# NethermindEth/latticefold

Hardware: AMD Instinct MI355X
Metric: folding-prover steps/sec (one NIFSProver::prove per step), GoldilocksRingNTT (higher is better)
Workload: dtype u64; 1 GPU; C4: GoldilocksRingNTT R1CS->CCS, m=N=2^20 rows, wit_len=262144, L=4, B=2^16, b=2, K=16, kappa=26, t=3; parallelism=replicas x1

## Files before the change

latticefold_amd/csrc/lf_common.h:

```cpp
#pragma once
#include <hip/hip_runtime.h>

#include <stdlib.h>

#include <atomic>

#include "../../include/lfhip.h"

#define HIPCHK(x)                                    \
    do {                                             \
        hipError_t e__ = (x);                        \
        if (e__ != hipSuccess) return LF_ERR_HIP;    \
    } while (0)
#define RET(x)                      \
    do {                            \
        int rc__ = (x);             \
        if (rc__ != LF_OK) return rc__; \
    } while (0)

extern "C" void lfplus_scratch_trim(int device);
template <class T> static inline hipError_t lf_dev_malloc(T **p, size_t bytes) {
    hipError_t e = hipMalloc((void **)p, bytes);
    if (e != hipErrorOutOfMemory) return e;
    (void)hipGetLastError();
    int dev = 0;
    if (hipGetDevice(&dev) != hipSuccess) return e;
    lfplus_scratch_trim(dev);
    return hipMalloc((void **)p, bytes);
}

struct DevBuf {
    void *p = nullptr;
    size_t bytes = 0;
    int ensure(size_t b) {
        if (b <= bytes) return LF_OK;
        if (p) (void)hipFree(p);
        p = nullptr;
        bytes = 0;
        const size_t slack = (b >> 3) < ((size_t)8 << 20) ? (b >> 3) : ((size_t)8 << 20);
        size_t want = b + slack + 256;
        if (hipMalloc(&p, want) != hipSuccess) {
            if (lf_dev_malloc(&p, b) != hipSuccess) return LF_ERR_HIP;
            want = b;
        }
        bytes = want;
        return LF_OK;
    }
    void release() {
        if (p) (void)hipFree(p);
        p = nullptr;
        bytes = 0;
    }
};

inline uint64_t lf_next_witness_id() {
    static std::atomic<uint64_t> next{1};
    return next.fetch_add(1, std::memory_order_relaxed);
}
struct lf_witness {
    lf_ctx *ctx;
    int32_t *planes;
    size_t N;
    int device;
    size_t plane_bytes;
    uint64_t id = lf_next_witness_id();
    uint64_t *f_ntt = nullptr;
    size_t f_bytes = 0;
    uint64_t *w_ccs = nullptr;
    size_t w_bytes = 0;
};

int lf_planes_alloc(lf_ctx *ctx, size_t bytes, int32_t **out);
void lf_planes_release(lf_ctx *ctx, size_t bytes, int32_t *p);
int lf_ctx_device(const lf_ctx *ctx);


struct Tunables {
    bool lin_u_eval = false, fold_unfused = false, fold_no_lut = false, fold_tab_r1 = false, theta_eval = false, fold_no_r4tab = false, fold_no_r5tab = false;
    bool fold_rounds_no_split = false;
    bool fold_sv_no_split = false;
    bool lin_no_split = false;
    size_t lin_split_min = (size_t)1 << 17;
    size_t fold_split_min = 8192;
    bool force_exchange = false;
    bool device_transcript = false;
    bool shard_plain_rounds = false;
    int shard_two_lanes = -1;
    size_t shard_lin_min = 16384;
    size_t shard_fold_min = 2048;
    long i8_wgs = 0;
    bool lin_no_r1cs = false;
    bool lin_no_small = false;
    size_t dot_min = 4096;
    bool dot_valu = false;
    bool fold_no_sv = false;
    size_t sv_min = 65536;
    int sv_rounds = 3;
    bool no_tail = false;
    size_t fuse_min = 16384, lut_min = (size_t)1 << 17, tab_min = 16384;
    size_t r5_min = 8192;
    size_t tail_n = 2048;
    static Tunables read(size_t lut_min_default) {
        Tunables t;
        t.lut_min = lut_min_default;
        const char *e;
        t.lin_u_eval = getenv("LF_LIN_U_EVAL") != nullptr;
        t.fold_unfused = getenv("LF_FOLD_UNFUSED") != nullptr;
        t.fold_no_lut = getenv("LF_FOLD_NO_LUT") != nullptr;
        t.fold_tab_r1 = getenv("LF_FOLD_TAB_R1") != nullptr;
        t.fold_no_r4tab = getenv("LF_FOLD_NO_R4TAB") != nullptr;
        t.fold_no_r5tab = getenv("LF_FOLD_NO_R5TAB") != nullptr;
        t.lin_no_split = getenv("LF_LIN_NO_SPLIT") != nullptr;
        t.fold_sv_no_split = getenv("LF_FOLD_SV_NO_SPLIT") != nullptr;
        t.fold_rounds_no_split = getenv("LF_FOLD_ROUNDS_NO_SPLIT") != nullptr;
        if (const char *e = getenv("LF_LIN_SPLIT_MIN")) t.lin_split_min = (size_t)atoll(e);
        if (const char *e = getenv("LF_FOLD_SPLIT_MIN")) t.fold_split_min = (size_t)atoll(e);
        t.theta_eval = getenv("LF_THETA_EVAL") != nullptr;
        t.no_tail = getenv("LF_NO_TAIL") != nullptr;
        t.fold_no_sv = getenv("LF_FOLD_NO_SV") != nullptr;
        t.dot_valu = getenv("LF_DOT_VALU") != nullptr;
        if ((e = getenv("LF_DOT_MIN"))) t.dot_min = (size_t)atoll(e);
        t.lin_no_small = getenv("LF_LIN_NO_SMALL") != nullptr;
        t.lin_no_r1cs = getenv("LF_LIN_NO_R1CS") != nullptr;
        if ((e = getenv("LF_FOLD_SV_MIN"))) t.sv_min = (size_t)atoll(e);
        if ((e = getenv("LF_FOLD_SV_ROUNDS"))) t.sv_rounds = atoi(e);
        if ((e = getenv("LF_I8_WGS"))) t.i8_wgs = atol(e);
        if ((e = getenv("LF_SHARD_TWO_LANES"))) t.shard_two_lanes = atoi(e) != 0;
        if ((e = getenv("LF_SHARD_LIN_MIN"))) t.shard_lin_min = (size_t)atoll(e);
        if ((e = getenv("LF_SHARD_FOLD_MIN"))) t.shard_fold_min = (size_t)atoll(e);
        t.shard_plain_rounds = getenv("LF_SHARD_PLAIN_ROUNDS") != nullptr;
        t.device_transcript = getenv("LF_DEVICE_TRANSCRIPT") != nullptr;
        t.force_exchange = getenv("LF_DIST_FORCE_EXCHANGE") != nullptr;
        if ((e = getenv("LF_FOLD_FUSE_MIN"))) t.fuse_min = (size_t)atoll(e);
        if ((e = getenv("LF_FOLD_LUT_MIN"))) t.lut_min = (size_t)atoll(e);
        if ((e = getenv("LF_FOLD_TAB_MIN"))) t.tab_min = (size_t)atoll(e);
        if ((e = getenv("LF_TAIL_N"))) t.tail_n = (size_t)atoll(e);
        if ((e = getenv("LF_FOLD_R5_MIN"))) t.r5_min = (size_t)atoll(e);
        return t;
    }
};

static inline int lf_validate_csr(unsigned t, size_t m, size_t n, const uint32_t *const *rowptr, const uint32_t *const *col,
                                  const uint64_t *const *val, int words, uint64_t modulus) {
    for (unsigned j = 0; j < t; j++) {
        if (!rowptr[j] || !col[j] || !val[j]) return LF_ERR_INVALID;
        if (rowptr[j][0] != 0) return LF_ERR_INVALID;
        for (size_t r = 0; r < m; r++)
            if (rowptr[j][r + 1] < rowptr[j][r]) return LF_ERR_INVALID;
        const size_t nnz = rowptr[j][m];
        for (size_t k = 0; k < nnz; k++)
            if (col[j][k] >= n) return LF_ERR_INVALID;
        for (size_t k = 0; k < nnz * (size_t)words; k++)
            if (val[j][k] >= modulus) return LF_ERR_INVALID;
    }
    return LF_OK;
}

struct ExtBasis {
    bool on = false;
    int tau = 0;
    uint64_t p = 0;
    uint64_t T[81], Ti[81];
    static uint64_t mulmod(uint64_t a, uint64_t b, uint64_t p) { return (uint64_t)(((unsigned __int128)a * b) % p); }
    void apply(const uint64_t *M, uint64_t *v) const {
        uint64_t o[9];
        for (int i = 0; i < tau; i++) {
            unsigned __int128 acc = 0;
            for (int j = 0; j < tau; j++) acc += (unsigned __int128)mulmod(M[i * tau + j], v[j], p);
            o[i] = (uint64_t)(acc % p);
        }
        for (int i = 0; i < tau; i++) v[i] = o[i];
    }
    void to_ext(uint64_t *v, size_t slots) const { if (on) for (size_t s = 0; s < slots; s++) apply(T, v + s * tau); }
    void to_int(uint64_t *v, size_t slots) const { if (on) for (size_t s = 0; s < slots; s++) apply(Ti, v + s * tau); }
    int set(const uint64_t *Tin, int tau_, uint64_t p_) {
        tau = tau_; p = p_;
        uint64_t M[9][18];
        bool ident = true;
        for (int i = 0; i < tau; i++)
            for (int j = 0; j < tau; j++) {
                uint64_t v = Tin[i * tau + j] % p;
                T[i * tau + j] = v; M[i][j] = v; M[i][tau + j] = i == j;
                if (v != (uint64_t)(i == j)) ident = false;
            }
        for (int i = 0; i < tau; i++)
            if (T[i * tau] != (uint64_t)(i == 0)) return LF_ERR_BAD_TABLES;
        auto inv = [&](uint64_t a) { uint64_t r = 1, e = p - 2; while (e) { if (e & 1) r = mulmod(r, a, p); a = mulmod(a, a, p); e >>= 1; } return r; };
        for (int c = 0; c < tau; c++) {
            int piv = -1;
            for (int r = c; r < tau; r++) if (M[r][c]) { piv = r; break; }
            if (piv < 0) return LF_ERR_BAD_TABLES;
            if (piv != c) for (int k = 0; k < 2 * tau; k++) { uint64_t t = M[piv][k]; M[piv][k] = M[c][k]; M[c][k] = t; }
            uint64_t iv = inv(M[c][c]);
            for (int k = 0; k < 2 * tau; k++) M[c][k] = mulmod(M[c][k], iv, p);
            for (int r = 0; r < tau; r++) {
                if (r == c || !M[r][c]) continue;
                uint64_t f = M[r][c];
                for (int k = 0; k < 2 * tau; k++) { uint64_t t = mulmod(f, M[c][k], p); M[r][k] = M[r][k] >= t ? M[r][k] - t : M[r][k] + (p - t); }
            }
        }
        for (int i = 0; i < tau; i++)
            for (int j = 0; j < tau; j++) Ti[i * tau + j] = M[i][tau + j];
// ... 5 lines not shown
```

latticefold_amd/csrc/lf_fold.cpp:

```cpp
#include "lf_ctx.h"

static int upload_consts(lf_ctx *c, const std::string &name, const std::vector<Fq3Const> &v, Fq3Const **out) {
    RET(c->tbuf(name, v.size() + 8, out));
    return c->h2d_small(*out, v.data(), v.size() * sizeof(Fq3Const));
}

static int tail_host_rounds(lf_ctx *c, Transcript &tr, u32 epoch, u32 nr, u32 npts, bool dev_transcript, u64 *msgs, Fq3 *pt,
                            const std::function<void(u32)> *after_round = nullptr, u32 round0 = 0) {
    TailMail *mail = c->tail_mail;
    const auto t_start = std::chrono::steady_clock::now();
    double host_us = 0, wait_us = 0;
    auto t_mark = t_start;
    const bool tl_on = t_tl && t_tl->on;
    for (u32 i = 0; i < nr; i++) {
        u32 spins = 0;
        while (__atomic_load_n(&mail->msg_seq[i], __ATOMIC_ACQUIRE) != epoch) {
            __builtin_ia32_pause();
            if ((++spins & 0xfff) == 0) {
                if (__atomic_load_n(&mail->err, __ATOMIC_RELAXED) == epoch ||
                    std::chrono::duration<double>(std::chrono::steady_clock::now() - t_start).count() > 10.0) {
                    __atomic_store_n(&mail->abort_seq, epoch, __ATOMIC_RELEASE);
                    (void)hipStreamSynchronize(c->stream());
                    return LF_ERR_HIP;
                }
// ... 83 lines not shown
    auto find = [&](unsigned s, unsigned b) {
        for (int i = 0; i < NPR; i++)
            if (prs[i].s == s && prs[i].b == b) return i;
        return -1;
    };
    std::vector<Fq3> wa(NX), wb(NX);
    for (int x = 0; x < NX; x++) {
        if (x < V) { wa[x] = W[x]; wb[x] = fq3_neg(W[x]); }
        else { wa[x] = fq3_zero(); wb[x] = W[x - V]; }
    }
    for (int x = 0; x < NX; x++)
        for (int y = x; y < NX; y++) {
            const Fq3 p2[3] = {c->ring.mul3(wa[x], wa[y]), fq3_add(c->ring.mul3(wa[x], wb[y]), c->ring.mul3(wb[x], wa[y])), c->ring.mul3(wb[x], wb[y])};
            for (int z = y; z < NX; z++) {
                Fq3 p3[4];
                p3[0] = c->ring.mul3(p2[0], wa[z]);
                p3[1] = fq3_add(c->ring.mul3(p2[0], wb[z]), c->ring.mul3(p2[1], wa[z]));
                p3[2] = fq3_add(c->ring.mul3(p2[1], wb[z]), c->ring.mul3(p2[2], wa[z]));
                p3[3] = c->ring.mul3(p2[2], wb[z]);
                int mult, idx;
                if (x == y && y == z) { mult = 1; idx = find(1u << x, 1u << x); }
                else if (x == y) { mult = 3; idx = find(1u << z, (1u << x) | (1u << z)); }
                else if (y == z) { mult = 3; idx = find(1u << x, (1u << x) | (1u << y)); }
                else { mult = 6; const unsigned mk = (1u << x) | (1u << y) | (1u << z); idx = find(mk, mk); }
                for (int e = 0; e < 4; e++) {
                    Fq3 t = p3[e], acc = fq3_zero();
                    for (int i = 0; i < mult; i++) acc = fq3_add(acc, t);
                    C[(size_t)idx * 4 + e] = fq3_add(C[(size_t)idx * 4 + e], acc);
                }
            }
        }
    for (int x = 0; x < NX; x++) {
        const int idx = find(1u << x, 1u << x);
        C[(size_t)idx * 4] = fq3_sub(C[(size_t)idx * 4], wa[x]);
        C[(size_t)idx * 4 + 1] = fq3_sub(C[(size_t)idx * 4 + 1], wb[x]);
    }
    out.resize((size_t)NPR * 12);
    for (size_t i = 0; i < (size_t)NPR * 4; i++)
        for (int q = 0; q < 3; q++) out[i * 3 + q] = C[i].c[q];
}

int fold_impl(lf_ctx *c, Transcript &tr, SideState *S , u64 *lcccs_out, lf_witness **w_out, u64 *proof) {
    const lf_params &P = c->P;
    size_t m = c->m, n = c->n, N = c->N;
    u32 K = P.K, K2 = 2 * K, deg = 2 * P.b;
    size_t ll = lf_lcccs_len(&P);
    std::vector<Fq3> alpha(K2), zeta(K2), mu(K2), beta(P.s);
    {
        HostTimer ht(c);
        tr.absorb_label("alpha_s");
        for (u32 i = 0; i < K2; i++) alpha[i] = tr.get_challenge();
        tr.absorb_label("zeta_s");
        for (u32 i = 0; i < K2; i++) zeta[i] = tr.get_challenge();
    }
    size_t ph = c->ev_begin(13);
    std::vector<Fq3Const> mu_pow((size_t)K2 * 3), a_pow((size_t)K2 * 3), z_pow((size_t)K2 * P.t);
    for (u32 i = 0; i < K2; i++) {
        Fq3 pa = alpha[i], pz = zeta[i];
        for (u32 d = 0; d < 3; d++) { a_pow[(size_t)i * 3 + d] = f3c(pa); pa = c->ring.mul3(pa, alpha[i]); }
        for (u32 j = 0; j < P.t; j++) { z_pow[(size_t)i * P.t + j] = f3c(pz); pz = c->ring.mul3(pz, zeta[i]); }
    }
    Fq3Const *d_mu, *d_ap, *d_zp;
    RET(upload_consts(c, "c_ap", a_pow, &d_ap));
    RET(upload_consts(c, "c_zp", z_pow, &d_zp));
    u64 *G[2], *eqb, *zz, *partial, *od;
    RET(c->tbuf("fold_G1", 24 * m, &G[0]));
    RET(c->tbuf("fold_G2", 24 * m, &G[1]));
    RET(c->tbuf("fold_eqb", 3 * m, &eqb));
    RET(c->tbuf("fold_zz", (size_t)P.t * 24 * n, &zz));
    RET(c->tbuf("round_partial", round_partial_words(), &partial));
    od = c->round_out();
    if (!od) return LF_ERR_HIP;
    u64 *const od_host = od, *od_shard = nullptr;
    if (c->sh_world > 1) {
        RET(c->tbuf("fold_round_out", 5 * 24 + 8, &od_shard));
        od = od_shard;
    }
    const bool shard_tabs = shard_keep(c, 1, m);
    const size_t g_r0 = shard_tabs ? (size_t)c->sh_rank * (m / (size_t)c->sh_world) : 0, g_rcnt = shard_tabs ? m / (size_t)c->sh_world : (size_t)-1;
    size_t zc_lo = 0, zc_hi = n;
    if (shard_tabs) RET(shard_col_range(c, g_r0, g_rcnt, &zc_lo, &zc_hi));
    {
        hipStream_t s0 = c->stream(), s1 = (t_lane == 0) ? c->st_lane[1] : s0;
        u64 *zz1 = zz;
        if (s1 != s0) {
            RET(c->tbuf("fold_zz1", (size_t)P.t * 24 * n, &zz1));
            if (!c->ev_prep[0]) { HIPCHK(hipEventCreateWithFlags(&c->ev_prep[0], hipEventDisableTiming)); HIPCHK(hipEventCreateWithFlags(&c->ev_prep[1], hipEventDisableTiming)); }
            HIPCHK(hipEventRecord(c->ev_prep[0], s0));
            HIPCHK(hipStreamWaitEvent(s1, c->ev_prep[0], 0));
        }
        for (int sd = 0; sd < 2; sd++) {
            hipStream_t st = sd ? s1 : s0;
            u64 *zb = sd ? zz1 : zz;
            launch_lincomb_z(c->dcrt, S[sd].z + zc_lo, n, K, d_zp + (size_t)sd * K * P.t, P.t, zc_hi - zc_lo, zb + zc_lo, st);
            if (c->ccs_general) {
                u64 *zaos;
                RET(c->tbuf(sd ? "spmv_zaos_R" : "spmv_zaos_L", (size_t)P.t * n * 24, &zaos));
                launch_spmv_rows(c->dcrt, P.t, c->d_rowptr.data(), c->d_col.data(), c->d_val.data(), zb, (size_t)24 * n, n, zaos, G[sd], m, 0, st, g_r0, g_rcnt);
            } else
            launch_spmv_sum(c->dcrt, P.t, c->d_rowptr.data(), c->d_col.data(), c->d_val.data(), zb, (size_t)24 * n, n, G[sd], m, st, g_r0, g_rcnt);
            launch_add_fhat_comb(c->dcrt, S[sd].planes, N, K, d_ap + (size_t)sd * K * 3, G[sd], m, st, g_r0, g_rcnt);
        }
        if (s1 != s0) {
            HIPCHK(hipEventRecord(c->ev_prep[1], s1));
            HIPCHK(hipStreamWaitEvent(s0, c->ev_prep[1], 0));
        }
    }
    {
        HostTimer ht(c);
        tr.absorb_label("mu_s");
        for (u32 i = 0; i + 1 < K2; i++) mu[i] = tr.get_challenge();
        mu[K2 - 1] = fq3_one();
        tr.absorb_label("beta_s");
        for (u32 i = 0; i < P.s; i++) beta[i] = tr.get_challenge();
    }
    TL_MARK(" fold challenges");
    for (u32 i = 0; i < K2; i++) {
        Fq3 pm = mu[i];
        for (u32 d = 0; d < 3; d++) { mu_pow[(size_t)i * 3 + d] = f3c(pm); pm = c->ring.mul3(pm, mu[i]); }
    }
    RET(upload_consts(c, "c_mu", mu_pow, &d_mu));
    RET(build_eq_dev(c, beta.data(), P.s, eqb));
    u64 *svE[3] = {nullptr, nullptr, nullptr};
    const bool sv_split = !c->tn.fold_sv_no_split && P.s >= 4 && m >= 256;
    if (sv_split) {
        RET(c->tbuf("fold_svE1", 3 * (m / 2), &svE[0]));
        RET(c->tbuf("fold_svE2", 3 * (m / 4), &svE[1]));
        RET(c->tbuf("fold_svE3", 3 * (m / 8), &svE[2]));
        RET(build_eq_dev(c, beta.data() + 1, P.s - 1, svE[0]));
    }
    Fq3 sv_c = fq3_one();
    u32 svE_level = 1;
    const bool fr_split = sv_split && c->sh_world == 1 && c->dcrt.nu2p40 && !c->tn.fold_rounds_no_split;
    u64 *svE_rest = nullptr;
    if (fr_split) RET(c->tbuf("fold_svE_rest", 3 * (m / 8) + 64, &svE_rest));
    auto svE_ptr = [&](u32 l) -> u64 * {
        if (l <= 3) return svE[l - 1];
        size_t off = 0;
        for (u32 q = 4; q < l; q++) off += 3 * (m >> q);
        return svE_rest + off;
    };
    auto svE_ensure = [&](u32 l) {
        for (; svE_level < l; svE_level++)
            launch_eq_pairsum(svE_ptr(svE_level), m >> svE_level, m >> (svE_level + 1), svE_ptr(svE_level + 1), m >> (svE_level + 1), c->stream());
    };
    auto sv_c_at = [&](u32 round, const std::vector<Fq3> &ptv) {
        Fq3 cc = fq3_one();
        for (u32 k = 1; k < round; k++) {
            const Fq3 b = beta[k - 1], r = ptv[k - 1];
            cc = c->ring.mul3(cc, fq3_add(c->ring.mul3(fq3_sub(fq3_one(), b), fq3_sub(fq3_one(), r)), c->ring.mul3(b, r)));
        }
        return cc;
    };
    LF_TRACE(c, "fold prepare");
    c->ev_end(ph);
    if (t_tl && t_tl->on) { (void)hipStreamSynchronize(c->stream()); TL_MARK(" fold prepare (synced)"); }

    ph = c->ev_begin(14);
    u64 *msgs = proof;
    std::vector<Fq3> pt(P.s);
    { HostTimer ht(c); sc_prologue(tr, P.s, deg); }
    const size_t Gw = (size_t)c->sh_world, gr = (size_t)c->sh_rank;
    bool sharded = Gw > 1;
    const bool fused = !c->tn.fold_unfused && (Gw == 1 || !c->tn.shard_plain_rounds);
    const size_t fuse_min = c->tn.fuse_min;
    int fmode = 0;
    const u64 *prevF = nullptr;
    size_t prevld = 0;
    const size_t lut_min = c->tn.lut_min;
    const size_t tab_min = c->tn.tab_min;
    const bool use_lut = fused && P.s >= 4 && m / 4 >= lut_min && m / 4 >= 4 && !c->tn.fold_no_lut;
    const bool use_r4tab = use_lut && c->dcrt.nu2p40 && !c->tn.fold_no_r4tab;
    const bool use_r5 = use_r4tab && !c->tn.fold_no_r5tab && Gw == 1 && P.s >= 5 && (N & 3) == 0 && (c->tn.no_tail || m / 8 > c->tn.tail_n) && m / 32 >= c->tn.r5_min;
    u64 *F[2], *T5[2];
    size_t half = m / 2;
    const size_t f0_ent = use_lut ? m / 16 : m / 4, f1_ent = use_r5 ? m / 32 : m / 8;
    RET(c->tbuf("fold_F0", (size_t)K2 * 3 * 24 * (f0_ent ? f0_ent : 1), &F[0]));
// ... 662 lines not shown
```

latticefold_amd/csrc/lf_kernels.h:

```cpp
#pragma once
#include "lf_ajtai_i8.h"
#include "lf_sv_rounds.h"
#include <hip/hip_runtime.h>

#include "lf_host.h"

namespace lf {

struct DevCrt {
    u64 nu;
    int nu2p40;
    u64 w4, w2, w10, w1, w7, w5, w11;
    int slot_of_pos[8], pos1[8], pos2[8];
    u64 tw1[8], tw2[8];
};
DevCrt make_dev_crt(const CrtTables &T);

struct Fq3Const { u64 c[3]; };

void launch_aos_to_soa(const u64 *aos, u64 *soa, size_t n, hipStream_t s);
void launch_soa_to_aos(const u64 *soa, u64 *aos, size_t n, hipStream_t s);
void launch_fill_uniform(u64 *dst, size_t words, u64 seed, size_t start, hipStream_t s);
void launch_fill_ajtai(u64 *A, u32 kappa, size_t n, size_t n_total, size_t col0, u64 seed, hipStream_t s, u32 row0 = 0);

void launch_modsum(const u64 *parts, u32 nparts, size_t words, u64 *out, hipStream_t s);
void launch_gather_relayout(const u64 *all, u32 nranks, size_t planes, size_t lcl, u64 *full, hipStream_t s);
void launch_gather_relayout_part(const u64 *all, u32 nranks, size_t planes_tot, size_t p0, size_t planes, size_t lcl, u64 *full, hipStream_t s);

void launch_selftest_field(u64 seed, u32 n, u64 *mism_dev, hipStream_t s);

void launch_crt_fwd(const DevCrt &t, const u64 *coef, u64 *ntt, size_t n, hipStream_t s);
void launch_icrt_dense(const u64 *icrt_mat , const u64 *ntt, u64 *coef, size_t n, hipStream_t s);


void launch_decompose(const u64 *coef, size_t n, u64 base, u32 digits, int layout, u64 *out, hipStream_t s, int mode = 0);
void launch_recompose(const u64 *in, size_t n_out, u64 base, u32 digits, u64 *out, hipStream_t s);
void launch_coef_to_i32(const u64 *coef, int32_t *planes, size_t n, u32 bound, int *viol, hipStream_t s);
void launch_i32_to_coef(const int32_t *planes, u64 *coef, size_t n, hipStream_t s);
void launch_recompose_crt(const DevCrt &t, const int32_t *planes, size_t n_planes, u32 wit_len, u32 L, u64 B, u32 K,
                          int mode_bits, u64 *out, size_t ldz, size_t off, hipStream_t s);
void launch_linf(const u64 *coef, size_t n, u64 *out_max, hipStream_t s);


void launch_build_eq(const DevCrt &t, const Fq3Const *r_dev , u32 nv, u64 *eq , hipStream_t s);
size_t build_eq_scratch_words(u32 nv);
void launch_build_eq2(const DevCrt &t, const Fq3Const *r_dev, u32 nv, u64 *scratch, u64 *eq, hipStream_t s);
void launch_spmv(const DevCrt &t, const u32 *rowptr, const u32 *col, const u64 *val , const u64 *z,
                 size_t ldz, u64 *out, size_t m, int accumulate, hipStream_t s, size_t r0 = 0, size_t rcnt = (size_t)-1 );
void launch_spmv_sum(const DevCrt &t, u32 nm, const u32 *const *rowptr, const u32 *const *col, const u64 *const *val, const u64 *z,
                     size_t z_stride, size_t ldz, u64 *out, size_t m, hipStream_t s, size_t r0 = 0, size_t rcnt = (size_t)-1 );
void launch_spmv_rows(const DevCrt &t, u32 nm, const u32 *const *rowptr, const u32 *const *col, const u64 *const *val, const u64 *z, size_t z_stride, size_t n,
                      u64 *zaos, u64 *out, size_t m, int accumulate, hipStream_t s, size_t r0 = 0, size_t rcnt = (size_t)-1);
void launch_spmv_t_eq(const DevCrt &t, const u32 *colptr, const u32 *rowidx, const u64 *val, const u64 *eq, size_t m,
                      u64 *q, size_t n, hipStream_t s, size_t c0 = 0, size_t ccnt = (size_t)-1 );
void launch_dot_batch(const DevCrt &t, const u64 *X, size_t ldx, u32 na, const u64 *Y, size_t ldy, u32 nb, size_t n,
                      u64 *partial, u64 *out, hipStream_t s);
size_t dot_partial_words(u32 na, u32 nb);
void launch_dot_eq(const DevCrt &t, const u64 *X, size_t ldx, u32 na, const u64 *eq, size_t ldeq, size_t n, u64 *partial,
                   u64 *out, hipStream_t s);
void launch_coef_eval(const DevCrt &t, const int32_t *planes, size_t n, const u64 *eq, size_t ldeq, u32 K, int mode_bits,
                      u64 *partial, u64 *out, hipStream_t s, size_t ldp = 0);
size_t coef_eval_partial_words(u32 K);
void launch_lincomb_z(const DevCrt &t, const u64 *z, size_t ldz, u32 K, const Fq3Const *coef_dev , u32 tt, size_t n,
                      u64 *out, hipStream_t s, u32 per_slot = 0);
void launch_add_fhat_comb(const DevCrt &t, const int32_t *planes, size_t n_planes, u32 K, const Fq3Const *apow_dev ,
                          u64 *G, size_t m, hipStream_t s, size_t r0 = 0, size_t rcnt = (size_t)-1 );

void launch_fix_ring(const DevCrt &t, const u64 *in, u64 *out, size_t n_in, Fq3Const r, hipStream_t s);
void launch_fix_fq3(const DevCrt &t, const u64 *in, u64 *out, size_t n_in, Fq3Const r, hipStream_t s);
size_t dot_i8_yb_bytes(size_t n);
size_t dot_i8_part_words(size_t n);
size_t dot_i8_tot_words();
int launch_dot_batch_i8(const DevCrt &t, const u64 *X, size_t ldx, u32 na, const u64 *Y, size_t ldy, u32 nb, size_t n, unsigned char *YB, int32_t *part,
                        long long *tot, u64 *out, hipStream_t s, bool y_packed = false, u32 nb_out = 0, u32 b0 = 0);
int launch_dot_pack_y(const u64 *X, const u64 *Y, size_t ldy, u32 nb, size_t n, unsigned char *YB, hipStream_t s);
void launch_vs_combine(const u64 *vs , u32 K, u64 *v , hipStream_t s);
void launch_fix_final(const DevCrt &t, const u64 *in , u32 rows3, Fq3Const r, u64 *out , hipStream_t s);

struct LinCombDesc {
    u32 t, q;
    u32 S_off[9];
    u32 S_idx[16];
    u64 c[8][24];
    int c_unit[8];
    u32 first[4];
    u32 ms[4];
};
void launch_lin_round(const DevCrt &t, const LinCombDesc &desc, const u64 *mz, size_t ld, const u64 *eq, size_t ldeq, size_t n,
                      u32 deg, u64 *partial, u64 *out, hipStream_t s, u32 max_blocks = 0, u32 split_xmask = 0 );
void launch_lin_round_fused(const DevCrt &t, const LinCombDesc &desc, const u64 *mz_prev, size_t ld_prev, const u64 *eq_prev, size_t ldeq_prev, Fq3Const r, u64 *mz_out,
                            size_t ld_out, u64 *eq_out, size_t ldeq_out, size_t n, u32 deg, u64 *partial, u64 *out, hipStream_t s, u32 max_blocks = 0,
                            u32 split_xmask = 0 );
void launch_eq_pairsum(const u64 *in, size_t ld_in, size_t n_out, u64 *out, size_t ld_out, hipStream_t s);
void launch_eq_expand(const DevCrt &t, const u64 *E, size_t lde, size_t pairs, Fq3Const w0, Fq3Const w1, u64 *out, size_t ldo, hipStream_t s);

struct FoldRoundArgs {
    const u64 *eqL, *eqR, *eqB;
    const u64 *G1, *G2;
    size_t ld;
    size_t n;
    size_t p0, pcnt;
    size_t pF0;
};
void launch_fold_round1(const DevCrt &t, const FoldRoundArgs &a, const int32_t *planesL, const int32_t *planesR, size_t n_planes,
                        u32 K, const Fq3Const *mu_pow_dev , u64 *partial, u64 *out, hipStream_t s);
void launch_fold_round_g(const DevCrt &t, const FoldRoundArgs &a, u64 *partial, u64 *out, hipStream_t s);
void launch_fold_materialize(const DevCrt &t, const int32_t *planesL, const int32_t *planesR, size_t n_planes, size_t m, u32 K,
                             Fq3Const r1, u64 *F, hipStream_t s);
void launch_fold_round2(const DevCrt &t, const FoldRoundArgs &a, const int32_t *planesL, const int32_t *planesR, size_t n_planes, u32 K,
                        const Fq3Const *mu_pow_dev, Fq3Const r1, u64 *partial, u64 *out, hipStream_t s);
void launch_fold_round_tab(const DevCrt &t, int round, const FoldRoundArgs &a, const int32_t *planesL, const int32_t *planesR, size_t n_planes, u32 K,
                           const Fq3Const *mu_pow_dev, const u64 *poly_dev, u64 *tp_dev, u64 *partial, u64 *out, hipStream_t s);
void launch_fold_materialize2(const DevCrt &t, const int32_t *planesL, const int32_t *planesR, size_t n_planes, size_t j0, size_t q, u32 K,
                              const Fq3Const W[4], u64 *F, hipStream_t s);
void launch_fold_round(const DevCrt &t, const FoldRoundArgs &a, const u64 *F, size_t ldF, u32 K, const Fq3Const *mu_pow_dev,
                       u64 *partial, u64 *out, hipStream_t s);
void launch_fold_round_lut_fix_tab(const DevCrt &t, const FoldRoundArgs &a, const int32_t *planesL, const int32_t *planesR, size_t n_planes,
                                   const u64 *lut_dev, Fq3Const r, u64 *sq_dev, u64 *mt_dev, u64 *Fout, size_t ldout, u32 K, const Fq3Const *mu_pow_dev,
                                   u64 *partial, u64 *out, hipStream_t s, const u64 *E = nullptr, size_t ldE = 0 );
void launch_fold_round_lut_fix5(const DevCrt &t, const FoldRoundArgs &a, const int32_t *planesL, const int32_t *planesR, size_t n_planes,
                                const u64 *lut_dev, Fq3Const r3, Fq3Const r4, u64 *xx_dev, u64 *yy_dev, u64 *mt_dev, u64 *Fout, size_t ldout, u32 K,
                                const Fq3Const *mu_pow_dev, u64 *partial, u64 *out, hipStream_t s, const u64 *E = nullptr, size_t ldE = 0 );
void launch_fold_round_fix(const DevCrt &t, const FoldRoundArgs &a, const u64 *Fprev, size_t ldprev, Fq3Const r, u64 *Fout, size_t ldout, u32 K,
                           const Fq3Const *mu_pow_dev, u64 *partial, u64 *out, hipStream_t s, const u64 *E = nullptr, size_t ldE = 0 );
void launch_fold_round_lut(const DevCrt &t, const FoldRoundArgs &a, const int32_t *planesL, const int32_t *planesR, size_t n_planes,
                           const u64 *lut_dev, u32 K, const Fq3Const *mu_pow_dev, u64 *partial, u64 *out, hipStream_t s);
void launch_fold_round_lut_mu(const DevCrt &t, const FoldRoundArgs &a, const int32_t *planesL, const int32_t *planesR, size_t n_planes,
                              const u64 *lut_dev, u64 *mutab_dev, u32 K, const Fq3Const *mu_pow_dev, u64 *partial, u64 *out, hipStream_t s);
void launch_fold_round_lut_fix(const DevCrt &t, const FoldRoundArgs &a, const int32_t *planesL, const int32_t *planesR, size_t n_planes,
                               const u64 *lut_dev, Fq3Const r, u64 *Fout, size_t ldout, u32 K, const Fq3Const *mu_pow_dev, u64 *partial,
                               u64 *out, hipStream_t s);
size_t round_partial_words();

void launch_sponge_script(const u64 *ark, const u64 *mds, const u32 *ops, u32 nops, const u64 *words, u64 *out, u64 *state_out, hipStream_t s);

constexpr u32 TAIL_MAX_ROUNDS = 32;
struct TailMail {
    u64 msg[TAIL_MAX_ROUNDS][128];
    u32 msg_seq[TAIL_MAX_ROUNDS];
    u64 chal[TAIL_MAX_ROUNDS][4];
    u32 chal_seq[TAIL_MAX_ROUNDS];
    u32 abort_seq;
    u32 err;
    u64 chal_out[TAIL_MAX_ROUNDS][4];
    u64 sponge[32];
    u64 dbg[TAIL_MAX_ROUNDS][8];
};
// ... 45 lines not shown
```

latticefold_amd/csrc/lf_kernels.hip:

```cpp
#include "lf_kernels.h"

#include <stdlib.h>

#include "lf_kernels_dev.cuh"

namespace lf {


DevCrt make_dev_crt(const CrtTables &T) {
    DevCrt d;
    d.nu = T.nu; d.nu2p40 = T.nu_is_2p40;
    d.w4 = T.w4; d.w2 = T.w2; d.w10 = T.w10; d.w1 = T.w1; d.w7 = T.w7; d.w5 = T.w5; d.w11 = T.w11;
    for (int p = 0; p < 8; p++) {
        d.slot_of_pos[p] = T.slot_of_pos[p]; d.pos1[p] = T.pos1[p]; d.pos2[p] = T.pos2[p];
        d.tw1[p] = T.tw1[p]; d.tw2[p] = T.tw2[p];
    }
    return d;
}


__device__ __forceinline__ u64 splitmix_fq(u64 seed, u64 index);


__global__ void __launch_bounds__(256) k_modsum(const u64 *parts, u32 nparts, size_t words, u64 *out) {
// ... 704 lines not shown
    __shared__ u64 red[3 * KG];
    block_sum_store<3 * KG>(acc, red);
    __syncthreads();
    if (threadIdx.x < 3 * KG) {
        u32 k = kg + threadIdx.x / 3, q = threadIdx.x % 3;
        if (k < K) partial[(size_t)blockIdx.x * (K * 72) + ((size_t)k * 24 + c) * 3 + q] = red[threadIdx.x];
    }
}
size_t coef_eval_partial_words(u32 K) { return (size_t)RED_BLOCKS * K * 72; }
void launch_coef_eval(const DevCrt &t, const int32_t *planes, size_t n, const u64 *eq, size_t ldeq, u32 K, int mode_bits, u64 *partial,
                      u64 *out, hipStream_t s, size_t ldp) {
    if (!ldp) ldp = n;
    u32 gb = (u32)((n + 255) / 256);
    if (gb > 64) gb = 64;
    if (gb < 1) gb = 1;
    static int kg = -1;
    if (kg < 0) kg = 8;
    if (mode_bits && kg == 16) hipLaunchKernelGGL(k_coef_eval<16>, dim3(gb, 24, (K + 15) / 16), dim3(256), 0, s, planes, ldp, n, eq, ldeq, K, mode_bits, partial);
    else if (mode_bits && kg == 8) hipLaunchKernelGGL(k_coef_eval<8>, dim3(gb, 24, (K + 7) / 8), dim3(256), 0, s, planes, ldp, n, eq, ldeq, K, mode_bits, partial);
    else hipLaunchKernelGGL(k_coef_eval<4>, dim3(gb, 24, mode_bits ? (K + 3) / 4 : 1), dim3(256), 0, s, planes, ldp, n, eq, ldeq, K, mode_bits, partial);
    hipLaunchKernelGGL(k_reduce_rows, dim3(K * 72), dim3(256), 0, s, partial, gb, K * 72, out);
}

template <bool NU, int TT>
__global__ void __launch_bounds__(256) k_lincomb_z(DevCrt t, const u64 *z, size_t ldz, u32 K, const Fq3Const *coef, size_t n, u64 *out, u32 per_slot) {
    size_t i = (size_t)blockIdx.x * 256 + threadIdx.x;
    u32 slot = blockIdx.y;
    if (i >= n) return;
    LH5 acc[TT];
    Fq3 accg[TT];
#pragma unroll
    for (int j = 0; j < TT; j++) { lh5_zero(acc[j]); accg[j] = fq3_zero(); }
    auto cf = [&](u32 k, int j) {
        Fq3Const cc = coef[per_slot ? (size_t)(k * TT + j) * 8 + slot : (size_t)(k * TT + j)];
        return fq3_make(cc.c[0], cc.c[1], cc.c[2]);
    };
    u32 k = 0;
    if (NU) {
        for (; k + 3 < K; k += 4) {
            Fq3 x[4], cv[4];
#pragma unroll
            for (int q = 0; q < 4; q++) x[q] = ld3(z + (size_t)(k + q) * 24 * ldz, ldz, slot, i);
#pragma unroll
            for (int j = 0; j < TT; j++) {
#pragma unroll
                for (int q = 0; q < 4; q++) cv[q] = cf(k + q, j);
                lh5_macn<4>(acc[j], x, cv);
            }
        }
        for (; k + 1 < K; k += 2) {
            Fq3 x0 = ld3(z + (size_t)k * 24 * ldz, ldz, slot, i), x1 = ld3(z + (size_t)(k + 1) * 24 * ldz, ldz, slot, i);
#pragma unroll
            for (int j = 0; j < TT; j++) lh5_mac2(acc[j], x0, cf(k, j), x1, cf(k + 1, j));
        }
    }
    for (; k < K; k++) {
        Fq3 x = ld3(z + (size_t)k * 24 * ldz, ldz, slot, i);
#pragma unroll
        for (int j = 0; j < TT; j++) {
            Fq3 cv = cf(k, j);
            if (NU) lh5_mac(acc[j], x, cv);
            else accg[j] = fq3_add(accg[j], M3<NU>(x, cv, t.nu));
        }
    }
#pragma unroll
    for (int j = 0; j < TT; j++) st3(out + (size_t)j * 24 * ldz, ldz, slot, i, NU ? lh5_finish(acc[j]) : accg[j]);
}
void launch_lincomb_z(const DevCrt &t, const u64 *z, size_t ldz, u32 K, const Fq3Const *coef_dev, u32 tt, size_t n, u64 *out, hipStream_t s, u32 per_slot) {
    if (!n) return;
#define LF_LZ(N)                                                                                                                              \
    do {                                                                                                                                      \
        if (t.nu2p40) hipLaunchKernelGGL((k_lincomb_z<true, N>), dim3(cdiv(n, 256), 8), dim3(256), 0, s, t, z, ldz, K, coef_dev, n, out, per_slot);    \
        else hipLaunchKernelGGL((k_lincomb_z<false, N>), dim3(cdiv(n, 256), 8), dim3(256), 0, s, t, z, ldz, K, coef_dev, n, out, per_slot);            \
    } while (0)
    switch (tt) {
        case 1: LF_LZ(1); break;
        case 2: LF_LZ(2); break;
        case 3: LF_LZ(3); break;
        default: LF_LZ(4); break;
    }
#undef LF_LZ
}

template <int NQ>
__global__ void __launch_bounds__(256) k_add_fhat_comb(const int32_t *planes, size_t n_planes, u32 K, const Fq3Const *apow, u64 *G, size_t m, size_t r0, size_t r1) {
    __shared__ u64 T[3 * NQ * 16][4];
    for (u32 e = threadIdx.x; e < 3 * NQ * 16; e += 256) {
        u32 val = e % 16, q = (e / 16) % NQ, d = e / (16 * NQ);
        Fq3 sum = fq3_zero();
        for (u32 b = 0; b < 4; b++)
            if (4 * q + b < K && ((val >> b) & 1)) {
                Fq3Const a = apow[(4 * q + b) * 3 + d];
                sum = fq3_add(sum, fq3_make(a.c[0], a.c[1], a.c[2]));
            }
        T[e][0] = sum.c[0]; T[e][1] = sum.c[1]; T[e][2] = sum.c[2]; T[e][3] = 0;
    }
    __syncthreads();
    size_t row = r0 + (size_t)blockIdx.x * 256 + threadIdx.x;
    u32 slot = blockIdx.y;
    if (row >= r1) return;
    Fq3 acc = ld3(G, m, slot, row);
#pragma unroll
    for (int d = 0; d < 3; d++) {
        int32_t v = planes[(size_t)(8 * d + slot) * n_planes + row];
        u32 mg = (u32)(v < 0 ? -v : v);
        Fq3 part = fq3_zero();
#pragma unroll
        for (int q = 0; q < NQ; q++) {
            const u64 *e = T[(d * NQ + q) * 16 + ((mg >> (4 * q)) & 15)];
            part = fq3_add(part, fq3_make(e[0], e[1], e[2]));
        }
        acc = v < 0 ? fq3_sub(acc, part) : fq3_add(acc, part);
    }
    st3(G, m, slot, row, acc);
}
void launch_add_fhat_comb(const DevCrt &t, const int32_t *planes, size_t n_planes, u32 K, const Fq3Const *apow_dev, u64 *G, size_t m,
                          hipStream_t s, size_t r0, size_t rcnt) {
    size_t r1 = rcnt == (size_t)-1 ? n_planes : (r0 + rcnt < n_planes ? r0 + rcnt : n_planes);
    if (rcnt == (size_t)-1) r0 = 0;
    if (r1 <= r0) return;
    if (K <= 16) hipLaunchKernelGGL(k_add_fhat_comb<4>, dim3(cdiv(r1 - r0, 256), 8), dim3(256), 0, s, planes, n_planes, K, apow_dev, G, m, r0, r1);
    else hipLaunchKernelGGL(k_add_fhat_comb<8>, dim3(cdiv(r1 - r0, 256), 8), dim3(256), 0, s, planes, n_planes, K, apow_dev, G, m, r0, r1);
}

template <bool NU>
__global__ void __launch_bounds__(256) k_fix(DevCrt t, const u64 *in, size_t ld_in, u64 *out, size_t ld_out, size_t n_out, Fq3Const r) {
    size_t j = (size_t)blockIdx.x * 256 + threadIdx.x;
    size_t row = blockIdx.y;
    if (j >= n_out) return;
    const u64 *p = in + row * 3 * ld_in;
    Fq3 rr = fq3_make(r.c[0], r.c[1], r.c[2]);
    ulonglong2 a0 = *(const ulonglong2 *)(p + 2 * j), a1 = *(const ulonglong2 *)(p + ld_in + 2 * j), a2 = *(const ulonglong2 *)(p + 2 * ld_in + 2 * j);
    Fq3 v0 = fq3_make(a0.x, a1.x, a2.x), v1 = fq3_make(a0.y, a1.y, a2.y);
    Fq3 res = fq3_add(v0, M3<NU>(fq3_sub(v1, v0), rr, t.nu));
    u64 *q = out + row * 3 * ld_out;
    q[j] = res.c[0]; q[ld_out + j] = res.c[1]; q[2 * ld_out + j] = res.c[2];
}
void launch_fix_ring(const DevCrt &t, const u64 *in, u64 *out, size_t n_in, Fq3Const r, hipStream_t s) {
    size_t n_out = n_in / 2;
    LF_LAUNCH(k_fix, t.nu2p40, dim3(cdiv(n_out, 256), 8), dim3(256), s, t, in, n_in, out, n_out, n_out, r);
}
void launch_fix_fq3(const DevCrt &t, const u64 *in, u64 *out, size_t n_in, Fq3Const r, hipStream_t s) {
    size_t n_out = n_in / 2;
    LF_LAUNCH(k_fix, t.nu2p40, dim3(cdiv(n_out, 256), 1), dim3(256), s, t, in, n_in, out, n_out, n_out, r);
}
void launch_fix_many(const DevCrt &t, const u64 *in, size_t ld_in, u64 *out, size_t ld_out, size_t n_in, u32 rows3, Fq3Const r, hipStream_t s) {
    size_t n_out = n_in / 2;
    LF_LAUNCH(k_fix, t.nu2p40, dim3(cdiv(n_out, 256), rows3), dim3(256), s, t, in, ld_in, out, ld_out, n_out, r);
}

template <bool NU>
__global__ void __launch_bounds__(256) k_fix_final(DevCrt t, const u64 *in, u32 rows3, Fq3Const r, u64 *out) {
    u32 row = blockIdx.x * 256 + threadIdx.x;
    if (row >= rows3) return;
    const u64 *p = in + (size_t)row * 6;
    Fq3 rr = fq3_make(r.c[0], r.c[1], r.c[2]);
    Fq3 v0 = fq3_make(p[0], p[2], p[4]), v1 = fq3_make(p[1], p[3], p[5]);
    Fq3 res = fq3_add(v0, M3<NU>(fq3_sub(v1, v0), rr, t.nu));
#pragma unroll
    for (int q = 0; q < 3; q++) out[(size_t)row * 3 + q] = fq_canon(res.c[q]);
}
__global__ void __launch_bounds__(128) k_vs_combine(const u64 *vs, u32 K, u64 *v) {
    const u32 i = threadIdx.x;
    if (i >= 72) return;
    u64 acc = 0, pw = 1;
    for (u32 k = 0; k < K; k++) {
// ... 80 lines not shown
```

Before: 59.63 steps/s.

## Compute fold witness linear combination directly from int32 decomposition planes

For the witness column range of z, the fold prepare step now builds the K-way linear combination straight from the compact signed int32 decomposition planes. It uses shared-memory nibble lookup tables over the coefficients, 96-bit accumulation and an in-register CRT/twist. Previously it read the full 24-word u64 NTT-domain z. This cuts memory traffic sharply for the dominant witness segment, at the cost of a more complex, compute-heavier kernel and extra launches for the head and tail ranges. An env flag restores the old path.

```diff
diff --git a/latticefold_amd/csrc/lf_common.h b/latticefold_amd/csrc/lf_common.h
--- a/latticefold_amd/csrc/lf_common.h
+++ b/latticefold_amd/csrc/lf_common.h
@@ -93,6 +93,7 @@
     bool lin_no_small = false;
     size_t dot_min = 4096;
     bool dot_valu = false;
+    bool fold_prepare_valu = false;
     bool fold_no_sv = false;
     size_t sv_min = 65536;
     int sv_rounds = 3;
@@ -118,6 +119,7 @@
         t.theta_eval = getenv("LF_THETA_EVAL") != nullptr;
         t.no_tail = getenv("LF_NO_TAIL") != nullptr;
         t.fold_no_sv = getenv("LF_FOLD_NO_SV") != nullptr;
+        t.fold_prepare_valu = getenv("LF_FOLD_PREPARE_VALU") != nullptr;
         t.dot_valu = getenv("LF_DOT_VALU") != nullptr;
         if ((e = getenv("LF_DOT_MIN"))) t.dot_min = (size_t)atoll(e);
         t.lin_no_small = getenv("LF_LIN_NO_SMALL") != nullptr;
diff --git a/latticefold_amd/csrc/lf_fold.cpp b/latticefold_amd/csrc/lf_fold.cpp
--- a/latticefold_amd/csrc/lf_fold.cpp
+++ b/latticefold_amd/csrc/lf_fold.cpp
@@ -189,6 +189,7 @@
     if (shard_tabs) RET(shard_col_range(c, g_r0, g_rcnt, &zc_lo, &zc_hi));
     {
         hipStream_t s0 = c->stream(), s1 = (t_lane == 0) ? c->st_lane[1] : s0;
+        const bool zz_planes = !c->tn.fold_prepare_valu && lincomb_planes_ok(K, P.L, P.t);
         u64 *zz1 = zz;
         if (s1 != s0) {
             RET(c->tbuf("fold_zz1", (size_t)P.t * 24 * n, &zz1));
@@ -196,10 +197,21 @@
             HIPCHK(hipEventRecord(c->ev_prep[0], s0));
             HIPCHK(hipStreamWaitEvent(s1, c->ev_prep[0], 0));
         }
+        const size_t hl = P.l + 1, w_end = hl + P.wit_len;
         for (int sd = 0; sd < 2; sd++) {
             hipStream_t st = sd ? s1 : s0;
             u64 *zb = sd ? zz1 : zz;
-            launch_lincomb_z(c->dcrt, S[sd].z + zc_lo, n, K, d_zp + (size_t)sd * K * P.t, P.t, zc_hi - zc_lo, zb + zc_lo, st);
+            const Fq3Const *zp = d_zp + (size_t)sd * K * P.t;
+            if (zz_planes) {
+                const size_t w_lo = zc_lo > hl ? zc_lo : hl, w_hi = zc_hi < w_end ? zc_hi : w_end, h_hi = zc_hi < hl ? zc_hi : hl, t_lo = zc_lo > w_end ? zc_lo : w_end;
+                const int32_t *const pls[2] = {S[sd].planes, nullptr};
+                const Fq3Const *const zps[2] = {zp, nullptr};
+                u64 *const zbs[2] = {zb, nullptr};
+                if (h_hi > zc_lo) launch_lincomb_z(c->dcrt, S[sd].z + zc_lo, n, K, zp, P.t, h_hi - zc_lo, zb + zc_lo, st);
+                if (zc_hi > t_lo) launch_lincomb_z(c->dcrt, S[sd].z + t_lo, n, K, zp, P.t, zc_hi - t_lo, zb + t_lo, st);
+                if (w_hi > w_lo) launch_lincomb_planes(c->dcrt, pls, N, P.L, P.B, K, zps, P.t, hl, w_lo, w_hi - w_lo, zbs, n, 1, st);
+            } else
+            launch_lincomb_z(c->dcrt, S[sd].z + zc_lo, n, K, zp, P.t, zc_hi - zc_lo, zb + zc_lo, st);
             if (c->ccs_general) {
                 u64 *zaos;
                 RET(c->tbuf(sd ? "spmv_zaos_R" : "spmv_zaos_L", (size_t)P.t * n * 24, &zaos));
diff --git a/latticefold_amd/csrc/lf_kernels.h b/latticefold_amd/csrc/lf_kernels.h
--- a/latticefold_amd/csrc/lf_kernels.h
+++ b/latticefold_amd/csrc/lf_kernels.h
@@ -63,6 +63,9 @@
 size_t coef_eval_partial_words(u32 K);
 void launch_lincomb_z(const DevCrt &t, const u64 *z, size_t ldz, u32 K, const Fq3Const *coef_dev , u32 tt, size_t n,
                       u64 *out, hipStream_t s, u32 per_slot = 0);
+bool lincomb_planes_ok(u32 K, u32 L, u32 tt);
+void launch_lincomb_planes(const DevCrt &t, const int32_t *const planes[2], size_t n_planes, u32 L, u64 B, u32 K, const Fq3Const *const coef_dev[2] ,
+                           u32 tt, size_t hl, size_t c0, size_t cnt, u64 *const out[2] , size_t ldz, int nsides, hipStream_t s);
 void launch_add_fhat_comb(const DevCrt &t, const int32_t *planes, size_t n_planes, u32 K, const Fq3Const *apow_dev ,
                           u64 *G, size_t m, hipStream_t s, size_t r0 = 0, size_t rcnt = (size_t)-1 );
 
diff --git a/latticefold_amd/csrc/lf_kernels.hip b/latticefold_amd/csrc/lf_kernels.hip
--- a/latticefold_amd/csrc/lf_kernels.hip
+++ b/latticefold_amd/csrc/lf_kernels.hip
@@ -810,6 +810,100 @@
 #undef LF_LZ
 }
 
+__device__ __forceinline__ void add_u96(u32 &l0, u32 &l1, u32 &h, u64 v) {
+    asm("v_add_co_u32 %0, vcc, %0, %3\n\tv_addc_co_u32 %1, vcc, %1, %4, vcc\n\tv_addc_co_u32 %2, vcc, 0, %2, vcc"
+        : "+v"(l0), "+v"(l1), "+v"(h) : "v"((u32)v), "v"((u32)(v >> 32)) : "vcc");
+}
+struct LincombPlanesSide { const int32_t *planes; const Fq3Const *coef ; u64 *out ; };
+struct LincombPlanesArgs { LincombPlanesSide sd[2]; size_t n_planes, ldz, c0, cnt; u32 hl, K, L, tt; u64 bpow[4], ntw[2][8] ; };
+template <bool L4>
+__global__ void __launch_bounds__(256) k_lincomb_planes(DevCrt t, LincombPlanesArgs a) {
+    __shared__ u64 T[3 * 4 * 4 * 32];
+    const u32 j = blockIdx.y;
+    const LincombPlanesSide sd = a.sd[blockIdx.z];
+    for (u32 e = threadIdx.x; e < 3 * 4 * 4 * 32; e += 256) {
+        const u32 nib = e & 15, neg = (e >> 4) & 1, q = (e >> 5) & 3, l = (e >> 7) & 3, ce = e >> 9;
+        u64 s = 0;
+        for (u32 b = 0; b < 4; b++)
+            if (4 * q + b < a.K && ((nib >> b) & 1)) s = fq_add(s, sd.coef[(size_t)(4 * q + b) * a.tt + j].c[ce]);
+        s = l < a.L ? fq_mul(s, a.bpow[l]) : 0;
+        T[e] = neg ? fq_neg(s) : s;
+    }
+    __syncthreads();
+    const size_t i = (size_t)blockIdx.x * 256 + threadIdx.x;
+    if (i >= a.cnt) return;
+    const size_t col = a.c0 + i, wi = col - a.hl;
+    u64 O[8][3];
+#pragma unroll
+    for (int p = 0; p < 8; p++) O[p][0] = O[p][1] = O[p][2] = 0;
+#pragma unroll 1
+    for (u32 u = 0; u < 3; u++) {
+        u64 x[3][8];
+#pragma unroll
+        for (int v8 = 0; v8 < 8; v8++) {
+            const int32_t *pl = sd.planes + (size_t)(3 * v8 + u) * a.n_planes + (size_t)a.L * wi;
+            int32_t v[4];
+            if (L4) {
+                const int4 w = *(const int4 *)pl;
+                v[0] = w.x; v[1] = w.y; v[2] = w.z; v[3] = w.w;
+            } else {
+#pragma unroll
+                for (int l = 0; l < 4; l++) v[l] = (u32)l < a.L ? pl[l] : 0;
+            }
+            u32 lo0[3] = {0, 0, 0}, lo1[3] = {0, 0, 0}, hi[3] = {0, 0, 0};
+#pragma unroll
+            for (int l = 0; l < 4; l++) {
+                const u32 mg = v[l] < 0 ? 0u - (u32)v[l] : (u32)v[l], sg = v[l] < 0 ? 16 : 0;
+#pragma unroll
+                for (int q = 0; q < 4; q++) {
+                    const u32 idx = ((l * 4 + q) << 5) + sg + ((mg >> (4 * q)) & 15);
+#pragma unroll
+                    for (int ce = 0; ce < 3; ce++) add_u96(lo0[ce], lo1[ce], hi[ce], T[ce * 512 + idx]);
+                }
+            }
+#pragma unroll
+            for (int ce = 0; ce < 3; ce++) x[ce][v8] = fq_add(fq_canon((u64)lo1[ce] << 32 | lo0[ce]), (u64)hi[ce] * LF_EPS);
+        }
+        u64 A[3][8];
+#pragma unroll
+        for (int ce = 0; ce < 3; ce++) crt8(x[ce], A[ce], t);
+#pragma unroll
+        for (int p = 0; p < 8; p++) {
+            if (u == 0) {
+                O[p][0] = fq_add(O[p][0], A[0][p]); O[p][1] = fq_add(O[p][1], A[1][p]); O[p][2] = fq_add(O[p][2], A[2][p]);
+            } else {
+                const bool c1 = (u == 1 ? t.pos1[p] : t.pos2[p]) == 1;
+                const u64 tw = u == 1 ? t.tw1[p] : t.tw2[p], ntw = a.ntw[u - 1][p];
+                const u64 r0 = fq_mul(tw, A[0][p]), r1 = fq_mul(c1 ? tw : ntw, A[1][p]), nr2 = fq_mul(ntw, A[2][p]);
+                O[p][0] = fq_add(O[p][0], c1 ? nr2 : r1);
+                O[p][1] = fq_add(O[p][1], c1 ? r0 : nr2);
+                O[p][2] = fq_add(O[p][2], c1 ? r1 : r0);
+            }
+        }
+    }
+    u64 *o = sd.out + (size_t)j * 24 * a.ldz + col;
+#pragma unroll
+    for (int p = 0; p < 8; p++) {
+        const size_t s3 = 3 * (size_t)t.slot_of_pos[p];
+        o[s3 * a.ldz] = O[p][0]; o[(s3 + 1) * a.ldz] = O[p][1]; o[(s3 + 2) * a.ldz] = O[p][2];
+    }
+}
+bool lincomb_planes_ok(u32 K, u32 L, u32 tt) { return K >= 1 && K <= 16 && L >= 1 && L <= 4 && tt >= 1 && tt <= 4; }
+void launch_lincomb_planes(const DevCrt &t, const int32_t *const planes[2], size_t n_planes, u32 L, u64 B, u32 K, const Fq3Const *const coef_dev[2], u32 tt,
+                           size_t hl, size_t c0, size_t cnt, u64 *const out[2], size_t ldz, int nsides, hipStream_t s) {
+    if (!cnt) return;
+    LincombPlanesArgs a;
+    for (int q = 0; q < 2; q++) a.sd[q] = {planes[q < nsides ? q : 0], coef_dev[q < nsides ? q : 0], out[q < nsides ? q : 0]};
+    a.n_planes = n_planes; a.ldz = ldz; a.c0 = c0; a.cnt = cnt; a.hl = (u32)hl; a.K = K; a.L = L; a.tt = tt;
+    u64 pw = 1;
+    for (int l = 0; l < 4; l++) { a.bpow[l] = pw; pw = fq_mul(pw, B % LF_P); }
+    for (int p = 0; p < 8; p++) { a.ntw[0][p] = fq_mul(t.nu, t.tw1[p]); a.ntw[1][p] = fq_mul(t.nu, t.tw2[p]); }
+    const bool l4 = L == 4 && (n_planes & 3) == 0 && ((uintptr_t)planes[0] & 15) == 0 && (nsides < 2 || ((uintptr_t)planes[1] & 15) == 0);
+    const dim3 g(cdiv(cnt, 256), tt, nsides);
+    if (l4) hipLaunchKernelGGL(k_lincomb_planes<true>, g, dim3(256), 0, s, t, a);
+    else hipLaunchKernelGGL(k_lincomb_planes<false>, g, dim3(256), 0, s, t, a);
+}
+
 template <int NQ>
 __global__ void __launch_bounds__(256) k_add_fhat_comb(const int32_t *planes, size_t n_planes, u32 K, const Fq3Const *apow, u64 *G, size_t m, size_t r0, size_t r1) {
     __shared__ u64 T[3 * NQ * 16][4];
```

Result: slower. 58.91 steps/s, median of 2 (-1.2%).
